# FortuneMU2025/LIDAR_AI_Recommendation_Software

Measured on AMD Instinct MI355X. Metric: M points/sec through SetAbstraction, 65k-pt frames; 1->8 GPU scaling, higher is better.
Workload: dtype f32

## Files before the change

lidar_ai_recommendation_software_amd/csrc/dense_x3s.hip:

```cpp
#include "h3.hpp"

int lidar_dense_x3_packed_image(int32_t k, int32_t cout, int64_t *bytes);

namespace {

using lidar_h3::f16x8;
typedef __bf16 bf16x8 __attribute__((ext_vector_type(8)));
typedef float f32x16 __attribute__((ext_vector_type(16)));
typedef float f32x4 __attribute__((ext_vector_type(4)));

#ifndef DENSE_SBK
#define DENSE_SBK 32
#endif
constexpr int SBM = 128, SBN = 128, SBK = DENSE_SBK;
constexpr int NSS = SBK / 16;
constexpr int CPR = SBK / 8;
constexpr int kStageA = SBM * SBK;
constexpr int kStageB = 4 * 2 * NSS * 512;
static_assert(SBK == 16 || SBK == 32, "DENSE_SBK must be 16 or 32");
__device__ __forceinline__ int swzf(int r) { return CPR == 4 ? (r >> 1) & 7 : (r >> 2) & 3; }


__device__ __forceinline__ f32x16 mfma_bf(bf16x8 a, bf16x8 b, f32x16 c)
{
    return __builtin_amdgcn_mfma_f32_32x32x16_bf16(a, b, c, 0, 0, 0);
}
__device__ __forceinline__ f32x16 mfma_h(f16x8 a, f16x8 b, f32x16 c)
{
    return __builtin_amdgcn_mfma_f32_32x32x16_f16(a, b, c, 0, 0, 0);
}

__device__ __forceinline__ void lds_dma16(const void *g, void *l)
{
    __builtin_amdgcn_global_load_lds((__attribute__((address_space(1))) void *)g,
                                     (__attribute__((address_space(3))) void *)l, 16, 0, 0);
}

using lidar::relu_nan;

template <int CTRL>
__device__ __forceinline__ float dpp_f(float v)
{
    return __int_as_float(__builtin_amdgcn_mov_dpp(__float_as_int(v), CTRL, 0xF, 0xF, true));
}
__device__ __forceinline__ float max_half_wave(float v)
{
    v = __builtin_elementwise_maximum(v, dpp_f<0xB1>(v));
    v = __builtin_elementwise_maximum(v, dpp_f<0x4E>(v));
    v = __builtin_elementwise_maximum(v, dpp_f<0x141>(v));
    v = __builtin_elementwise_maximum(v, dpp_f<0x140>(v));
    const auto b = __builtin_amdgcn_permlane16_swap(__float_as_uint(v), __float_as_uint(v), false, false);
    return __builtin_elementwise_maximum(v, __builtin_elementwise_maximum(__uint_as_float(b[0]), __uint_as_float(b[1])));
}

__device__ __forceinline__ bf16x8 round8_bf(const f32x4 &a0, const f32x4 &a1)
{
    bf16x8 hi;
#pragma unroll
    for (int j = 0; j < 8; ++j) hi[j] = (__bf16)(j < 4 ? a0[j] : a1[j - 4]);
    return hi;
}

__device__ __forceinline__ int swzp(int r) { return CPR == 4 ? (r >> 2) & 3 : (r >> 3) & 1; }

__device__ __forceinline__ int out_bound_exp(float colsum, float bmax, int e_in)
{
    const float b = (colsum * ldexpf(1.0f, e_in) + bmax) * (1.0f + 0x1p-10f);
    return lidar_h3::exp_of_bits(__float_as_uint(b));
}

template <int MODE, bool X1, bool PL = false>
__global__ __launch_bounds__(256, 2) void dense_x3_kernel(const float *__restrict__ af, int lda,
                                                          const uint16_t *__restrict__ wp, int ks,
                                                          const int32_t *__restrict__ wexp,
                                                          const float *__restrict__ bias, int relu_on,
                                                          int pool_rows, float *__restrict__ out, int64_t ldo,
                                                          int cout, int ntn, int64_t total, int64_t per_xcd, int kdim,
                                                          const int32_t *__restrict__ a_exp = nullptr,
                                                          int64_t a_plane = 0, int32_t *__restrict__ out_exp = nullptr,
                                                          float w_colsum = 0.0f, float b_max = 0.0f)
{
    static_assert(!PL || !X1, "h3 planes carry the fp32 contract only");
    static_assert(MODE != 1 || !X1, "mode 1 writes h3 planes");
    __shared__ __attribute__((aligned(16))) float As0[kStageA], As1[kStageA];
    __shared__ __attribute__((aligned(16))) uint16_t Bs0[kStageB], Bs1[kStageB];
    auto Asb = [&](int buf) { return buf ? As1 : As0; };
    auto Bsb = [&](int buf) { return buf ? Bs1 : Bs0; };
    const int tid = threadIdx.x, lane = tid & 63, wave = __builtin_amdgcn_readfirstlane(tid >> 6);
    const int h = lane >> 5, col = lane & 31;
    const int64_t L = blockIdx.x;
    const int64_t logical = (L & 7) * per_xcd + (L >> 3);
    if (logical >= total) return;
    const int64_t row0 = logical / ntn * SBM;
    const int tn = (int)(logical % ntn);
    const int nst = (kdim + SBK - 1) / SBK;

    auto load_stage = [&](int st, int buf) {
        const int k0 = st * SBK;
        if constexpr (PL) {
            constexpr int RPI = 64 / CPR;
            const int pl = wave >> 1, rbase = 64 * (wave & 1);
            const uint16_t *ap = reinterpret_cast<const uint16_t *>(af) + pl * a_plane;
            uint16_t *dst = reinterpret_cast<uint16_t *>(Asb(buf)) + pl * (SBM * SBK);
#pragma unroll
            for (int t = 0; t < CPR; ++t) {
                const int r = rbase + RPI * t + lane / CPR;
                const int q = (lane % CPR) ^ swzp(r);
                lds_dma16(ap + (row0 + r) * lda + k0 + 8 * q, dst + (rbase + RPI * t) * SBK);
            }
        } else {
        constexpr int CF = 2 * CPR, RPI = 64 / CF;
        float *dst = Asb(buf);
#pragma unroll
        for (int i = 0; i < CPR; ++i) {
            const int r = 32 * wave + RPI * i + lane / CF;
            const int kq = (lane % CF) ^ swzf(r);
            const int kc = k0 + 4 * kq < kdim ? k0 + 4 * kq : k0;
            lds_dma16(af + (row0 + r) * lda + kc, dst + (32 * wave + RPI * i) * SBK);
        }
        }
        const uint16_t *src = wp + (((int64_t)(4 * tn + wave) * ks + NSS * st) * 2) * 512;
#pragma unroll
        for (int i = 0; i < 2 * NSS; ++i) lds_dma16(src + i * 512 + lane * 8, &Bsb(buf)[(wave * 2 * NSS + i) * 512]);
        __builtin_amdgcn_sched_barrier(0);
    };

    f32x16 acc[4] = {};
    int E = lidar_h3::kEmin - 1;
    if constexpr (PL) E = a_exp[row0 + 32 * wave + col];
    auto frag = [&](const float *as, int ss, f32x4 &a0, f32x4 &a1) {
        const int r = 32 * wave + col;
        const int kq = 4 * ss + 2 * h;
        const int sl = kq ^ swzf(r);
        a0 = *reinterpret_cast<const f32x4 *>(as + r * SBK + 4 * sl);
        a1 = *reinterpret_cast<const f32x4 *>(as + r * SBK + 4 * (sl ^ 1));
    };
    auto compute = [&](int buf) {
        if constexpr (PL) {
            const uint16_t *ah = reinterpret_cast<const uint16_t *>(Asb(buf));
            const int r = 32 * wave + col;
#pragma unroll
            for (int ss = 0; ss < NSS; ++ss) {
                const int slot = (2 * ss + h) ^ swzp(r);
                const f16x8 xh = *reinterpret_cast<const f16x8 *>(ah + (r * CPR + slot) * 8);
                const f16x8 xl = *reinterpret_cast<const f16x8 *>(ah + SBM * SBK + (r * CPR + slot) * 8);
#pragma unroll
                for (int j = 0; j < 4; ++j) {
                    const f16x8 wh = *reinterpret_cast<const f16x8 *>(&Bsb(buf)[((j * NSS + ss) * 2 + 0) * 512 + lane * 8]);
                    const f16x8 wl = *reinterpret_cast<const f16x8 *>(&Bsb(buf)[((j * NSS + ss) * 2 + 1) * 512 + lane * 8]);
                    acc[j] = mfma_h(wh, xh, acc[j]);
                    acc[j] = mfma_h(wl, xh, acc[j]);
                    acc[j] = mfma_h(wh, xl, acc[j]);
                }
            }
            return;
        }
        const float *as = Asb(buf);
        float S = 1.0f;
        if constexpr (!X1) {
            float m = 0.0f;
#pragma unroll
            for (int ss = 0; ss < NSS; ++ss) {
                f32x4 a0, a1;
                frag(as, ss, a0, a1);
#pragma unroll
                for (int t = 0; t < 4; ++t) m = lidar_h3::absmax3(m, a0[t], a1[t]);
            }
            const auto sw32 = __builtin_amdgcn_permlane32_swap(__float_as_uint(m), __float_as_uint(m), false, false);
            m = lidar_h3::absmax3(m, __uint_as_float(sw32[0]), __uint_as_float(sw32[1]));
            const int e = lidar_h3::exp_of_bits(__float_as_uint(m)) + 3;
            if (__ballot(e > E)) {
                const int d = e > E ? E - e : 0;
#pragma unroll
                for (int j = 0; j < 4; ++j)
#pragma unroll
                    for (int r = 0; r < 16; ++r) acc[j][r] = ldexpf(acc[j][r], d);
                E = e > E ? e : E;
            }
            S = lidar_h3::scale_of(E);
            asm volatile("" ::: "memory");
        }
#pragma unroll
        for (int ss = 0; ss < NSS; ++ss) {
            f32x4 a0, a1;
            frag(as, ss, a0, a1);
            if constexpr (X1) {
                const bf16x8 xh = round8_bf(a0, a1);
#pragma unroll
                for (int j = 0; j < 4; ++j) {
                    const bf16x8 wh = *reinterpret_cast<const bf16x8 *>(&Bsb(buf)[((j * NSS + ss) * 2 + 0) * 512 + lane * 8]);
                    acc[j] = mfma_bf(wh, xh, acc[j]);
                }
            } else {
                f16x8 xh, xl;
                lidar_h3::split8(a0, a1, S, xh, xl);
#pragma unroll
                for (int j = 0; j < 4; ++j) {
                    const f16x8 wh = *reinterpret_cast<const f16x8 *>(&Bsb(buf)[((j * NSS + ss) * 2 + 0) * 512 + lane * 8]);
                    const f16x8 wl = *reinterpret_cast<const f16x8 *>(&Bsb(buf)[((j * NSS + ss) * 2 + 1) * 512 + lane * 8]);
                    acc[j] = mfma_h(wh, xh, acc[j]);
                    acc[j] = mfma_h(wl, xh, acc[j]);
                    acc[j] = mfma_h(wh, xl, acc[j]);
                }
            }
        }
    };
    load_stage(0, 0);
    for (int st = 0; st < nst; st += 2) {
        __syncthreads();
        if (st + 1 < nst) load_stage(st + 1, 1);
        compute(0);
        if (st + 1 < nst) {
            __syncthreads();
            if (st + 2 < nst) load_stage(st + 2, 0);
            compute(1);
        }
    }
    if (wexp[1] != (X1 ? lidar_h3::kTagX1 : lidar_h3::kTagH3)) {
#pragma unroll
        for (int j = 0; j < 4; ++j)
#pragma unroll
            for (int r = 0; r < 16; ++r) acc[j][r] = __builtin_nanf("");
    }
    if constexpr (!X1) {
        const int us = E - 14 - *wexp;
#pragma unroll
        for (int j = 0; j < 4; ++j)
#pragma unroll
            for (int r = 0; r < 16; ++r) acc[j][r] = ldexpf(acc[j][r], us);
    }
    const int cbase = tn * SBN;
    if constexpr (MODE == 1) {
        const int64_t row = row0 + 32 * wave + col;
        const int eo = out_bound_exp(w_colsum, b_max, PL ? E : E - 3);
        const float so = lidar_h3::scale_of(eo);
        uint16_t *oh = reinterpret_cast<uint16_t *>(out);
#pragma unroll
        for (int j = 0; j < 4; ++j)
#pragma unroll
            for (int g = 0; g < 4; ++g) {
                const int c = cbase + 32 * j + 8 * g + 4 * h;
                const f32x4 b4 = *reinterpret_cast<const f32x4 *>(bias + c);
                float v[4];
#pragma unroll
                for (int t = 0; t < 4; ++t) {
                    const float y = acc[j][4 * g + t] + b4[t];
                    v[t] = (relu_on ? relu_nan(y) : y) * so;
                }
                uint32_t hi[2], lo[2];
                lidar_h3::split2(v[0], v[1], hi[0], lo[0]);
                lidar_h3::split2(v[2], v[3], hi[1], lo[1]);
                *reinterpret_cast<uint2 *>(oh + row * ldo + c) = make_uint2(hi[0], hi[1]);
                *reinterpret_cast<uint2 *>(oh + row * ldo + c + (int64_t)total / ntn * SBM * ldo) = make_uint2(lo[0], lo[1]);
            }
        if (h == 0 && tn == 0) out_exp[row] = eo;
    } else if constexpr (MODE == 0) {
        const int64_t row = row0 + 32 * wave + col;
#pragma unroll
        for (int j = 0; j < 4; ++j)
#pragma unroll
            for (int g = 0; g < 4; ++g) {
                const int c = cbase + 32 * j + 8 * g + 4 * h;
                const f32x4 b4 = *reinterpret_cast<const f32x4 *>(bias + c);
                f32x4 v;
#pragma unroll
                for (int t = 0; t < 4; ++t) {
                    const float y = acc[j][4 * g + t] + b4[t];
                    v[t] = relu_on ? relu_nan(y) : y;
                }
                *reinterpret_cast<f32x4 *>(out + row * ldo + c) = v;
            }
    } else {
        unsigned *orow = reinterpret_cast<unsigned *>(out + (row0 / pool_rows) * ldo);
#pragma unroll
        for (int j = 0; j < 4; ++j) {
            float mine = 0.0f;
#pragma unroll
            for (int r = 0; r < 16; ++r) {
                const float v = max_half_wave(acc[j][r]);
                mine = col == r ? v : mine;
            }
            if (col < 16) {
                const int c = cbase + 32 * j + 8 * (col >> 2) + 4 * h + (col & 3);
                atomicMax(orow + c, __float_as_uint(relu_nan(mine + bias[c])));
            }
        }
    }
}

int launch_dense_x3(const char *fn, lidar_handle *h, const float *a, int32_t lda, int64_t rows, int32_t k,
                    const int32_t *a_exp, int64_t a_plane, const void *packed, const float *bias, int32_t cout,
                    int32_t mode, bool x1, int32_t relu_on, int32_t pool_rows, float *out, int32_t *out_exp,
                    int64_t ldo, float w_colsum, float b_max, void *stream)
{
    REQUIRE(ldo >= cout && ldo % 4 == 0, std::string(fn) + ": ldo must be >= cout and a multiple of 4");
    REQUIRE(mode != 2 || (relu_on && pool_rows > 0 && pool_rows % SBM == 0 && rows % pool_rows == 0),
            std::string(fn) + ": the max-pool needs relu and pool_rows a multiple of 128 dividing rows");
    if (rows == 0) return LIDAR_OK;
    ON_DEVICE(h->device);
    const int ks = (k + 31) / 32 * 2;
    const int ntn = cout / SBN;
    const int64_t total = (rows / SBM) * ntn, per_xcd = (total + 7) / 8;
    REQUIRE(per_xcd * 8 <= 0x7fffffff, std::string(fn) + ": too many rows");
    int64_t wbytes = 0;
    if (lidar_dense_x3_packed_image(k, cout, &wbytes) != LIDAR_OK) return LIDAR_EINVAL;
    hipStream_t s = static_cast<hipStream_t>(stream);
    const uint16_t *w = static_cast<const uint16_t *>(packed);
    const int32_t *wexp = reinterpret_cast<const int32_t *>(static_cast<const char *>(packed) + wbytes);
    const dim3 grid((unsigned)(per_xcd * 8)), block(256);
    const int rl = relu_on ? 1 : 0;
    auto go = [&](auto kern, int relu, int pool) {
        hipLaunchKernelGGL(kern, grid, block, 0, s, a, (int)lda, w, ks, wexp, bias, relu, pool, out, ldo, (int)cout, ntn,
                           total, per_xcd, (int)k, a_exp, a_plane, out_exp, w_colsum, b_max);
    };
    const bool pl = a_exp != nullptr;
    if (x1) go(dense_x3_kernel<0, true>, rl, 0);
    else if (!pl && mode == 0) go(dense_x3_kernel<0, false>, rl, 0);
    else if (!pl && mode == 2) go(dense_x3_kernel<2, false>, 1, (int)pool_rows);
    else if (pl && mode == 0) go(dense_x3_kernel<0, false, true>, rl, 0);
    else if (pl && mode == 1) go(dense_x3_kernel<1, false, true>, rl, 0);
    else if (pl) go(dense_x3_kernel<2, false, true>, 1, (int)pool_rows);
    else go(dense_x3_kernel<1, false>, rl, 0);
    LAUNCH_CHECK();
    return LIDAR_OK;
}

}

LIDAR_EXPORT int lidar_dense_x3f_f32(lidar_handle *h, const float *a, int32_t lda, int64_t rows, int32_t k,
                                     const void *packed, const float *bias, int32_t cout, int32_t mode,
                                     int32_t relu_on, int32_t pool_rows, void *out, int64_t o_plane, int64_t ldo,
                                     void *stream)
{
    const bool x1 = (mode & 4) != 0;
    mode &= 3;
    (void)o_plane;
    REQUIRE(!x1 || mode == 0, "lidar_dense_x3f_f32: the X1 flag needs mode 0");
    REQUIRE(h && a && packed && bias && out, "lidar_dense_x3f_f32: null pointer");
    REQUIRE(rows % SBM == 0 && k > 0 && k <= lda && cout % SBN == 0 && cout > 0,
            "lidar_dense_x3f_f32: rows % 128, k <= lda, cout % 128 must hold");
    REQUIRE(k % 4 == 0 && lda % 4 == 0, "lidar_dense_x3f_f32: k % 4 == 0 and lda % 4 == 0 (fp32 rows)");
    REQUIRE(mode == 0 || mode == 2, "lidar_dense_x3f_f32: mode must be 0 or 2");
    return launch_dense_x3("lidar_dense_x3f_f32", h, a, lda, rows, k, nullptr, 0, packed, bias, cout, mode, x1, relu_on,
                           pool_rows, static_cast<float *>(out), nullptr, ldo, 0.0f, 0.0f, stream);
}

LIDAR_EXPORT int lidar_dense_h3p_f32(lidar_handle *h, const void *a, int32_t lda, int64_t rows, int32_t k,
                                     const int32_t *a_exp, const void *packed, const float *bias, int32_t cout,
                                     int32_t mode, int32_t relu_on, int32_t pool_rows, void *out, int32_t *out_exp,
                                     int64_t ldo, float w_colsum, float b_max, void *stream)
{
    REQUIRE(h && a && packed && bias && out, "lidar_dense_h3p_f32: null pointer");
    REQUIRE(rows % SBM == 0 && k > 0 && k <= lda && cout % SBN == 0 && cout > 0,
            "lidar_dense_h3p_f32: rows % 128, k <= lda, cout % 128 must hold");
    REQUIRE(a_exp != nullptr ? lda == (k + 31) / 32 * 32 : (k % 4 == 0 && lda % 4 == 0),
            "lidar_dense_h3p_f32: planes need lda = k rounded up to 32; fp32 rows k % 4 == 0 and lda % 4 == 0");
    REQUIRE(mode >= 0 && mode <= 2, "lidar_dense_h3p_f32: mode must be 0, 1 or 2");
    REQUIRE(mode != 1 || (out_exp != nullptr && ldo == cout && w_colsum >= 0.0f && b_max >= 0.0f),
            "lidar_dense_h3p_f32: mode 1 needs out_exp, ldo == cout and the bounds w_colsum, b_max >= 0");
    return launch_dense_x3("lidar_dense_h3p_f32", h, static_cast<const float *>(a), lda, rows, k, a_exp, rows * lda,
                           packed, bias, cout, mode, false, relu_on, pool_rows, static_cast<float *>(out), out_exp,
                           ldo, w_colsum, b_max, stream);
}
```

Before: 1285.

## Pipeline LDS weight fragments, stage bias in LDS, transposed pooled epilogue, phase stamps

In the h3-plane path, all activation fragments for a stage are now loaded up front, and the weight fragments are double-buffered in registers so the next LDS read overlaps the current MFMAs. For the pooled mode, operands are swapped so the max-pool reduces over registers before the atomics, and the per-row unscale is folded into that epilogue. Bias is loaded once early and staged through LDS for the epilogue. The fp32 path skips the second substep when the K tail is 16 or less. Optional LIDAR_DIAG s_memtime phase stamps are added, and they compile out by default.

Measured after the change: 1286 (median of 4 runs). No clear change (+0.1%).

```diff
diff --git a/lidar_ai_recommendation_software_amd/csrc/dense_x3s.hip b/lidar_ai_recommendation_software_amd/csrc/dense_x3s.hip
--- a/lidar_ai_recommendation_software_amd/csrc/dense_x3s.hip
+++ b/lidar_ai_recommendation_software_amd/csrc/dense_x3s.hip
@@ -36,6 +36,27 @@
                                      (__attribute__((address_space(3))) void *)l, 16, 0, 0);
 }
 
+#ifdef LIDAR_DIAG
+#define DENSE_DIAG_TPARAM , bool DIAG = false
+#define DENSE_DIAG_ARG , uint64_t *diag = nullptr
+#define DENSE_DIAG_NULL , static_cast<uint64_t *>(nullptr)
+#define DENSE_STAMP(...) \
+    if constexpr (DIAG) { __VA_ARGS__ }
+__device__ __forceinline__ uint64_t stamp()
+{
+    uint64_t t;
+    __builtin_amdgcn_sched_barrier(0);
+    asm volatile("s_memtime %0\n\ts_waitcnt lgkmcnt(0)" : "=s"(t)::"memory");
+    __builtin_amdgcn_sched_barrier(0);
+    return t;
+}
+#else
+#define DENSE_DIAG_TPARAM
+#define DENSE_DIAG_ARG
+#define DENSE_DIAG_NULL
+#define DENSE_STAMP(...)
+#endif
+
 using lidar::relu_nan;
 
 template <int CTRL>
@@ -69,7 +90,7 @@
     return lidar_h3::exp_of_bits(__float_as_uint(b));
 }
 
-template <int MODE, bool X1, bool PL = false>
+template <int MODE, bool X1, bool PL = false DENSE_DIAG_TPARAM>
 __global__ __launch_bounds__(256, 2) void dense_x3_kernel(const float *__restrict__ af, int lda,
                                                           const uint16_t *__restrict__ wp, int ks,
                                                           const int32_t *__restrict__ wexp,
@@ -78,10 +99,11 @@
                                                           int cout, int ntn, int64_t total, int64_t per_xcd, int kdim,
                                                           const int32_t *__restrict__ a_exp = nullptr,
                                                           int64_t a_plane = 0, int32_t *__restrict__ out_exp = nullptr,
-                                                          float w_colsum = 0.0f, float b_max = 0.0f)
+                                                          float w_colsum = 0.0f, float b_max = 0.0f DENSE_DIAG_ARG)
 {
     static_assert(!PL || !X1, "h3 planes carry the fp32 contract only");
     static_assert(MODE != 1 || !X1, "mode 1 writes h3 planes");
+    constexpr bool POOLT = MODE == 2 && PL;
     __shared__ __attribute__((aligned(16))) float As0[kStageA], As1[kStageA];
     __shared__ __attribute__((aligned(16))) uint16_t Bs0[kStageB], Bs1[kStageB];
     auto Asb = [&](int buf) { return buf ? As1 : As0; };
@@ -125,6 +147,19 @@
         __builtin_amdgcn_sched_barrier(0);
     };
 
+    const int cbase = tn * SBN;
+    float bq[2] = {0.0f, 0.0f};
+    if constexpr (POOLT) {
+        bq[0] = bias[cbase + 32 * h + col];
+        bq[1] = bias[cbase + 32 * (2 + h) + col];
+    } else if constexpr (MODE != 2) {
+        const float2 b2 = *reinterpret_cast<const float2 *>(bias + cbase + 2 * lane);
+        bq[0] = b2.x;
+        bq[1] = b2.y;
+    }
+#ifdef LIDAR_DIAG
+    uint64_t dt[5] = {}, tl = 0;
+#endif
     f32x16 acc[4] = {};
     int E = lidar_h3::kEmin - 1;
     if constexpr (PL) E = a_exp[row0 + 32 * wave + col];
@@ -135,15 +170,82 @@
         a0 = *reinterpret_cast<const f32x4 *>(as + r * SBK + 4 * sl);
         a1 = *reinterpret_cast<const f32x4 *>(as + r * SBK + 4 * (sl ^ 1));
     };
-    auto compute = [&](int buf) {
+    auto compute = [&](int buf, int st) {
         if constexpr (PL) {
             const uint16_t *ah = reinterpret_cast<const uint16_t *>(Asb(buf));
             const int r = 32 * wave + col;
+            f16x8 xh[NSS], xl[NSS], wh[2], wl[2];
+            auto wfrag = [&](int t, int set) {
+                const int ss = t >> 2, j = t & 3;
+                wh[set] = *reinterpret_cast<const f16x8 *>(&Bsb(buf)[((j * NSS + ss) * 2 + 0) * 512 + lane * 8]);
+                wl[set] = *reinterpret_cast<const f16x8 *>(&Bsb(buf)[((j * NSS + ss) * 2 + 1) * 512 + lane * 8]);
+            };
 #pragma unroll
             for (int ss = 0; ss < NSS; ++ss) {
                 const int slot = (2 * ss + h) ^ swzp(r);
-                const f16x8 xh = *reinterpret_cast<const f16x8 *>(ah + (r * CPR + slot) * 8);
-                const f16x8 xl = *reinterpret_cast<const f16x8 *>(ah + SBM * SBK + (r * CPR + slot) * 8);
+                xh[ss] = *reinterpret_cast<const f16x8 *>(ah + (r * CPR + slot) * 8);
+                xl[ss] = *reinterpret_cast<const f16x8 *>(ah + SBM * SBK + (r * CPR + slot) * 8);
+            }
+            wfrag(0, 0);
+#pragma unroll
+            for (int t = 0; t < 4 * NSS; ++t) {
+                const int ss = t >> 2, j = t & 3, set = t & 1;
+                if (t + 1 < 4 * NSS) wfrag(t + 1, set ^ 1);
+                __builtin_amdgcn_sched_barrier(0);
+                if constexpr (POOLT) {
+                    acc[j] = mfma_h(xh[ss], wh[set], acc[j]);
+                    acc[j] = mfma_h(xh[ss], wl[set], acc[j]);
+                    acc[j] = mfma_h(xl[ss], wh[set], acc[j]);
+                } else {
+                    acc[j] = mfma_h(wh[set], xh[ss], acc[j]);
+                    acc[j] = mfma_h(wl[set], xh[ss], acc[j]);
+                    acc[j] = mfma_h(wh[set], xl[ss], acc[j]);
+                }
+            }
+            return;
+        }
+        const float *as = Asb(buf);
+        const int nss = X1 || kdim - st * SBK > 16 ? NSS : 1;
+        float S = 1.0f;
+        if constexpr (!X1) {
+            float m = 0.0f;
+#pragma unroll
+            for (int ss = 0; ss < NSS; ++ss) {
+                if (ss >= nss) break;
+                f32x4 a0, a1;
+                frag(as, ss, a0, a1);
+#pragma unroll
+                for (int t = 0; t < 4; ++t) m = lidar_h3::absmax3(m, a0[t], a1[t]);
+            }
+            const auto sw32 = __builtin_amdgcn_permlane32_swap(__float_as_uint(m), __float_as_uint(m), false, false);
+            m = lidar_h3::absmax3(m, __uint_as_float(sw32[0]), __uint_as_float(sw32[1]));
+            const int e = lidar_h3::exp_of_bits(__float_as_uint(m)) + 3;
+            if (__ballot(e > E)) {
+                const int d = e > E ? E - e : 0;
+#pragma unroll
+                for (int j = 0; j < 4; ++j)
+#pragma unroll
+                    for (int r = 0; r < 16; ++r) acc[j][r] = ldexpf(acc[j][r], d);
+                E = e > E ? e : E;
+            }
+            S = lidar_h3::scale_of(E);
+            asm volatile("" ::: "memory");
+        }
+#pragma unroll
+        for (int ss = 0; ss < NSS; ++ss) {
+            if (ss >= nss) break;
+            f32x4 a0, a1;
+            frag(as, ss, a0, a1);
+            if constexpr (X1) {
+                const bf16x8 xh = round8_bf(a0, a1);
+#pragma unroll
+                for (int j = 0; j < 4; ++j) {
+                    const bf16x8 wh = *reinterpret_cast<const bf16x8 *>(&Bsb(buf)[((j * NSS + ss) * 2 + 0) * 512 + lane * 8]);
+                    acc[j] = mfma_bf(wh, xh, acc[j]);
+                }
+            } else {
+                f16x8 xh, xl;
+                lidar_h3::split8(a0, a1, S, xh, xl);
 #pragma unroll
                 for (int j = 0; j < 4; ++j) {
                     const f16x8 wh = *reinterpret_cast<const f16x8 *>(&Bsb(buf)[((j * NSS + ss) * 2 + 0) * 512 + lane * 8]);
@@ -153,67 +255,22 @@
                     acc[j] = mfma_h(wh, xl, acc[j]);
                 }
             }
-            return;
-        }
-        const float *as = Asb(buf);
-        float S = 1.0f;
-        if constexpr (!X1) {
-            float m = 0.0f;
-#pragma unroll
-            for (int ss = 0; ss < NSS; ++ss) {
-                f32x4 a0, a1;
-                frag(as, ss, a0, a1);
-#pragma unroll
-                for (int t = 0; t < 4; ++t) m = lidar_h3::absmax3(m, a0[t], a1[t]);
-            }
-            const auto sw32 = __builtin_amdgcn_permlane32_swap(__float_as_uint(m), __float_as_uint(m), false, false);
-            m = lidar_h3::absmax3(m, __uint_as_float(sw32[0]), __uint_as_float(sw32[1]));
-            const int e = lidar_h3::exp_of_bits(__float_as_uint(m)) + 3;
-            if (__ballot(e > E)) {
-                const int d = e > E ? E - e : 0;
-#pragma unroll
-                for (int j = 0; j < 4; ++j)
-#pragma unroll
-                    for (int r = 0; r < 16; ++r) acc[j][r] = ldexpf(acc[j][r], d);
-                E = e > E ? e : E;
-            }
-            S = lidar_h3::scale_of(E);
-            asm volatile("" ::: "memory");
-        }
-#pragma unroll
-        for (int ss = 0; ss < NSS; ++ss) {
-            f32x4 a0, a1;
-            frag(as, ss, a0, a1);
-            if constexpr (X1) {
-                const bf16x8 xh = round8_bf(a0, a1);
-#pragma unroll
-                for (int j = 0; j < 4; ++j) {
-                    const bf16x8 wh = *reinterpret_cast<const bf16x8 *>(&Bsb(buf)[((j * NSS + ss) * 2 + 0) * 512 + lane * 8]);
-                    acc[j] = mfma_bf(wh, xh, acc[j]);
-                }
-            } else {
-                f16x8 xh, xl;
-                lidar_h3::split8(a0, a1, S, xh, xl);
-#pragma unroll
-                for (int j = 0; j < 4; ++j) {
-                    const f16x8 wh = *reinterpret_cast<const f16x8 *>(&Bsb(buf)[((j * NSS + ss) * 2 + 0) * 512 + lane * 8]);
-                    const f16x8 wl = *reinterpret_cast<const f16x8 *>(&Bsb(buf)[((j * NSS + ss) * 2 + 1) * 512 + lane * 8]);
-                    acc[j] = mfma_h(wh, xh, acc[j]);
-                    acc[j] = mfma_h(wl, xh, acc[j]);
-                    acc[j] = mfma_h(wh, xl, acc[j]);
-                }
-            }
         }
     };
+    DENSE_STAMP(dt[0] = dt[4] = stamp();)
     load_stage(0, 0);
     for (int st = 0; st < nst; st += 2) {
         __syncthreads();
+        DENSE_STAMP(const uint64_t t = stamp(); if (st == 0) dt[0] = t - dt[0]; else dt[1] += t - tl; tl = t;)
         if (st + 1 < nst) load_stage(st + 1, 1);
-        compute(0);
+        compute(0, st);
+        DENSE_STAMP(const uint64_t t = stamp(); dt[2] += t - tl; tl = t;)
         if (st + 1 < nst) {
             __syncthreads();
+            DENSE_STAMP(const uint64_t t = stamp(); dt[1] += t - tl; tl = t;)
             if (st + 2 < nst) load_stage(st + 2, 0);
-            compute(1);
+            compute(1, st + 1);
+            DENSE_STAMP(const uint64_t t = stamp(); dt[2] += t - tl; tl = t;)
         }
     }
     if (wexp[1] != (X1 ? lidar_h3::kTagX1 : lidar_h3::kTagH3)) {
@@ -222,25 +279,34 @@
 #pragma unroll
             for (int r = 0; r < 16; ++r) acc[j][r] = __builtin_nanf("");
     }
-    if constexpr (!X1) {
+    if constexpr (!X1 && !POOLT) {
         const int us = E - 14 - *wexp;
 #pragma unroll
         for (int j = 0; j < 4; ++j)
 #pragma unroll
             for (int r = 0; r < 16; ++r) acc[j][r] = ldexpf(acc[j][r], us);
     }
-    const int cbase = tn * SBN;
+    const float *bs = nullptr;
+    if constexpr (MODE != 2) {
+        float *bw = As0 + 32 * wave * (PL ? SBK / 2 : SBK);
+        *reinterpret_cast<float2 *>(bw + 2 * lane) = make_float2(bq[0], bq[1]);
+        bs = bw;
+    }
     if constexpr (MODE == 1) {
         const int64_t row = row0 + 32 * wave + col;
         const int eo = out_bound_exp(w_colsum, b_max, PL ? E : E - 3);
         const float so = lidar_h3::scale_of(eo);
         uint16_t *oh = reinterpret_cast<uint16_t *>(out);
 #pragma unroll
-        for (int j = 0; j < 4; ++j)
+        for (int j = 0; j < 4; ++j) {
+            f32x4 bj[4];
+#pragma unroll
+            for (int g = 0; g < 4; ++g) bj[g] = *reinterpret_cast<const f32x4 *>(bs + 32 * j + 8 * g + 4 * h);
+            __builtin_amdgcn_sched_barrier(0);
 #pragma unroll
             for (int g = 0; g < 4; ++g) {
                 const int c = cbase + 32 * j + 8 * g + 4 * h;
-                const f32x4 b4 = *reinterpret_cast<const f32x4 *>(bias + c);
+                const f32x4 b4 = bj[g];
                 float v[4];
 #pragma unroll
                 for (int t = 0; t < 4; ++t) {
@@ -253,15 +319,20 @@
                 *reinterpret_cast<uint2 *>(oh + row * ldo + c) = make_uint2(hi[0], hi[1]);
                 *reinterpret_cast<uint2 *>(oh + row * ldo + c + (int64_t)total / ntn * SBM * ldo) = make_uint2(lo[0], lo[1]);
             }
+        }
         if (h == 0 && tn == 0) out_exp[row] = eo;
     } else if constexpr (MODE == 0) {
         const int64_t row = row0 + 32 * wave + col;
 #pragma unroll
-        for (int j = 0; j < 4; ++j)
+        for (int j = 0; j < 4; ++j) {
+            f32x4 bj[4];
+#pragma unroll
+            for (int g = 0; g < 4; ++g) bj[g] = *reinterpret_cast<const f32x4 *>(bs + 32 * j + 8 * g + 4 * h);
+            __builtin_amdgcn_sched_barrier(0);
 #pragma unroll
             for (int g = 0; g < 4; ++g) {
                 const int c = cbase + 32 * j + 8 * g + 4 * h;
-                const f32x4 b4 = *reinterpret_cast<const f32x4 *>(bias + c);
+                const f32x4 b4 = bj[g];
                 f32x4 v;
 #pragma unroll
                 for (int t = 0; t < 4; ++t) {
@@ -270,6 +341,27 @@
                 }
                 *reinterpret_cast<f32x4 *>(out + row * ldo + c) = v;
             }
+        }
+    } else if constexpr (POOLT) {
+        unsigned *orow = reinterpret_cast<unsigned *>(out + (row0 / pool_rows) * ldo);
+        const int us = E - 14 - *wexp;
+        f32x4 m;
+#pragma unroll
+        for (int r = 0; r < 16; ++r) {
+            const int ur = __shfl(us, 8 * (r >> 2) + 4 * h + (r & 3));
+            const f32x4 v = {ldexpf(acc[0][r], ur), ldexpf(acc[1][r], ur), ldexpf(acc[2][r], ur), ldexpf(acc[3][r], ur)};
+            m = r == 0 ? v : __builtin_elementwise_maximum(m, v);
+        }
+#pragma unroll
+        for (int j = 0; j < 4; ++j) {
+            const auto b = __builtin_amdgcn_permlane32_swap(__float_as_uint(m[j]), __float_as_uint(m[j]), false, false);
+            m[j] = __builtin_elementwise_maximum(m[j], __builtin_elementwise_maximum(__uint_as_float(b[0]), __uint_as_float(b[1])));
+        }
+#pragma unroll
+        for (int jj = 0; jj < 2; ++jj) {
+            const float v = h ? m[2 * jj + 1] : m[2 * jj];
+            atomicMax(orow + cbase + 32 * (2 * jj + h) + col, __float_as_uint(relu_nan(v + bq[jj])));
+        }
     } else {
         unsigned *orow = reinterpret_cast<unsigned *>(out + (row0 / pool_rows) * ldo);
 #pragma unroll
@@ -286,12 +378,18 @@
             }
         }
     }
+    DENSE_STAMP(const uint64_t t = stamp(); dt[3] = t - tl; dt[4] = t - dt[4];
+                if (lane == 0) {
+                    uint64_t *d = diag + (L * 4 + wave) * 6;
+                    for (int i = 0; i < 5; ++i) d[i] = dt[i];
+                    d[5] = (uint64_t)nst;
+                })
 }
 
 int launch_dense_x3(const char *fn, lidar_handle *h, const float *a, int32_t lda, int64_t rows, int32_t k,
                     const int32_t *a_exp, int64_t a_plane, const void *packed, const float *bias, int32_t cout,
                     int32_t mode, bool x1, int32_t relu_on, int32_t pool_rows, float *out, int32_t *out_exp,
-                    int64_t ldo, float w_colsum, float b_max, void *stream)
+                    int64_t ldo, float w_colsum, float b_max, void *stream DENSE_DIAG_ARG)
 {
     REQUIRE(ldo >= cout && ldo % 4 == 0, std::string(fn) + ": ldo must be >= cout and a multiple of 4");
     REQUIRE(mode != 2 || (relu_on && pool_rows > 0 && pool_rows % SBM == 0 && rows % pool_rows == 0),
@@ -311,9 +409,24 @@
     const int rl = relu_on ? 1 : 0;
     auto go = [&](auto kern, int relu, int pool) {
         hipLaunchKernelGGL(kern, grid, block, 0, s, a, (int)lda, w, ks, wexp, bias, relu, pool, out, ldo, (int)cout, ntn,
-                           total, per_xcd, (int)k, a_exp, a_plane, out_exp, w_colsum, b_max);
+                           total, per_xcd, (int)k, a_exp, a_plane, out_exp, w_colsum, b_max DENSE_DIAG_NULL);
     };
     const bool pl = a_exp != nullptr;
+#ifdef LIDAR_DIAG
+    if (diag) {
+        auto god = [&](auto kern, int relu, int pool) {
+            hipLaunchKernelGGL(kern, grid, block, 0, s, a, (int)lda, w, ks, wexp, bias, relu, pool, out, ldo, (int)cout,
+                               ntn, total, per_xcd, (int)k, a_exp, a_plane, out_exp, w_colsum, b_max, diag);
+        };
+        REQUIRE(!x1 && (pl ? mode != 0 : mode != 2), std::string(fn) + ": no stamped instantiation of this form");
+        if (!pl && mode == 0) god(dense_x3_kernel<0, false, false, true>, rl, 0);
+        else if (!pl) god(dense_x3_kernel<1, false, false, true>, rl, 0);
+        else if (mode == 1) god(dense_x3_kernel<1, false, true, true>, rl, 0);
+        else god(dense_x3_kernel<2, false, true, true>, 1, (int)pool_rows);
+        LAUNCH_CHECK();
+        return LIDAR_OK;
+    }
+#endif
     if (x1) go(dense_x3_kernel<0, true>, rl, 0);
     else if (!pl && mode == 0) go(dense_x3_kernel<0, false>, rl, 0);
     else if (!pl && mode == 2) go(dense_x3_kernel<2, false>, 1, (int)pool_rows);
@@ -362,3 +475,22 @@
                            packed, bias, cout, mode, false, relu_on, pool_rows, static_cast<float *>(out), out_exp,
                            ldo, w_colsum, b_max, stream);
 }
+
+#ifdef LIDAR_DIAG
+LIDAR_EXPORT int lidar_diag_dense_phases(lidar_handle *h, const void *a, int32_t lda, int64_t rows, int32_t k,
+                                         const int32_t *a_exp, const void *packed, const float *bias, int32_t cout,
+                                         int32_t mode, int32_t relu_on, int32_t pool_rows, void *out, int32_t *out_exp,
+                                         int64_t ldo, float w_colsum, float b_max, uint64_t *diag, void *stream)
+{
+    REQUIRE(h && a && packed && bias && out && diag, "lidar_diag_dense_phases: null pointer");
+    REQUIRE(rows % SBM == 0 && k > 0 && k <= lda && cout % SBN == 0 && cout > 0,
+            "lidar_diag_dense_phases: rows % 128, k <= lda, cout % 128 must hold");
+    REQUIRE(a_exp != nullptr ? lda == (k + 31) / 32 * 32 : (k % 4 == 0 && lda % 4 == 0),
+            "lidar_diag_dense_phases: planes need lda = k rounded up to 32; fp32 rows k % 4 == 0 and lda % 4 == 0");
+    REQUIRE(mode >= 0 && mode <= 2 && (mode != 1 || (out_exp != nullptr && ldo == cout)),
+            "lidar_diag_dense_phases: mode 0, 1 (with out_exp, ldo == cout) or 2");
+    return launch_dense_x3("lidar_diag_dense_phases", h, static_cast<const float *>(a), lda, rows, k, a_exp, rows * lda,
+                           packed, bias, cout, mode, false, relu_on, pool_rows, static_cast<float *>(out), out_exp,
+                           ldo, w_colsum, b_max, stream, diag);
+}
+#endif
```
